# CLIAI/speaker-diarization-toolkit

Hardware: AMD Instinct MI355X
Metric: segment-embeddings/sec (higher is better)
Workload: dtype bf16; 1 GPU; config #2: 1k synthetic 2-s segments/GPU -> fbank -> ECAPA-TDNN C=1024 -> L2 -> cosine argmax vs 100 profiles; segments_per_gpu=1000, embed_dim=192, weights=random-init seed 0 (20.77 M params), parallelism=segments sharded x1, profiles replicated

## Files before the change

speaker-diarization-toolkit_amd/csrc/common.hpp:

```cpp
#pragma once
#include <hip/hip_runtime.h>
#include <stdint.h>
#include <stdio.h>
#include <vector>

#include "../../include/sdk_hip.h"

typedef __bf16 bf16_t;
typedef __bf16 bf16x8 __attribute__((ext_vector_type(8)));
typedef __bf16 bf16x4 __attribute__((ext_vector_type(4)));
typedef __bf16 bf16x2 __attribute__((ext_vector_type(2)));
typedef float f32x4 __attribute__((ext_vector_type(4)));
typedef float f32x16 __attribute__((ext_vector_type(16)));
typedef uint32_t u32x4 __attribute__((ext_vector_type(4)));
typedef uint32_t u32x2 __attribute__((ext_vector_type(2)));

struct sdk_prof_rec {
  int family;
  hipEvent_t a, b;
  double flops, bytes;
};
struct sdk_ctx {
  int device;
  int num_cu;
  hipDeviceProp_t prop;
  bool prof_on = false;
  bool no_chain_fusion = false;
  bool no_chain_two_per_cu = false;
  bool no_chain_packed = false;
  bool no_asp_packed = false;
  bool no_asp_seg = false;
  bool no_h_kblocked = false;
  int precision = 0;
  int aff_fast = 1;
  void* dbg_ptr = nullptr;
  void* gemm_clk_ptr = nullptr;
  void* gemm_stamps_ptr = nullptr;
  int hp_gemm_variant = 0;
  int matvec_variant = 0;
  int aff_boundary_pen = 0;
  int chol_pivot_rtol_ppb = 1000;
  int chol_shift_ppb = 0;
  bool ahc_distances_only = false;
  bool snorm_scores_only = false;
  int aff_variant = 0;
  std::vector<const void*> lds_optin;
  std::vector<sdk_prof_rec> prof;
};

int sdk_lds_optin(sdk_ctx* ctx, const void* func, int bytes);

int asp_fused_launch(sdk_ctx* ctx, const uint16_t* ah, int64_t ldah, const uint16_t* w2, const uint16_t* w2p, const float* b2,
                     const uint16_t* h, int64_t ldh, int B, int T, int C, int A, float* pooled, void* stream, bool kblocked = false, bool f16 = false);

int se_gate_residual_impl(sdk_ctx* ctx, const uint16_t* z, int64_t ldz, const uint16_t* x, int64_t ldx, const float* w1t, const float* b1, const float* w2t,
                          const float* b2, uint16_t* out, int64_t ldo, int B, int T, int C, int Cse, const float* mean_in, void* ws, size_t ws_bytes,
                          void* stream, bool f16);
int asp_stats_impl(sdk_ctx* ctx, const uint16_t* h, int64_t ldh, int B, int T, int C, float* out_ctx, void* stream, bool f16);
int asp_pool_impl(sdk_ctx* ctx, const float* logits, int64_t ldl, const uint16_t* h, int64_t ldh, int B, int T, int C, float* pooled, void* stream, bool f16);

int res2net_chain_launch(sdk_ctx* ctx, const uint16_t* U, int64_t ldu, uint16_t* R, int64_t ldr, const uint16_t* const* W,
                         const uint16_t* const* Wpk, const float* const* bias, const float* const* scale, const float* const* shift,
                         int nconv, int B, int T, int dil, void* stream, bool f16 = false);

int resnet_tstp_impl(sdk_ctx* ctx, const uint16_t* x, int B, int F, int T, int C, float* out, void* stream, bool f16);
int resnet_masked_tstp_impl(sdk_ctx* ctx, const uint16_t* x, int B, int F, int T, int C, int S, const float* w, const int32_t* valid, float* out,
                            void* stream, bool f16);
int resnet_zero_invalid_impl(sdk_ctx* ctx, float* emb, int n, int dim, const int32_t* valid, void* stream);

size_t ahc_workspace_bytes(const int32_t* offsets, int G);
int ahc_launch(sdk_ctx* ctx, const float* E, int ldE, int dim, const int32_t* offsets, int G, double* Z, int32_t* status, void* ws, void* stream);

struct ProfScope {
  sdk_ctx* c; hipStream_t s; size_t slot; bool on;
  ProfScope(sdk_ctx* ctx, void* stream, int family, double flops, double bytes) : c(ctx), s((hipStream_t)stream), slot(0), on(ctx && ctx->prof_on) {
    if (!on) return;
    sdk_prof_rec r{family, nullptr, nullptr, flops, bytes};
    (void)hipEventCreate(&r.a); (void)hipEventCreate(&r.b);
    (void)hipEventRecord(r.a, s);
    slot = c->prof.size();
    c->prof.push_back(r);
  }
  ~ProfScope() { if (on) (void)hipEventRecord(c->prof[slot].b, s); }
};

void sdk_set_error(const char* fmt, ...) __attribute__((format(printf, 1, 2)));

#define SDK_HIP_OK(expr)                                                              \
  do {                                                                                \
    hipError_t _e = (expr);                                                           \
    if (_e != hipSuccess) {                                                           \
      sdk_set_error("%s failed: %s (%s:%d)", #expr, hipGetErrorString(_e), __FILE__, __LINE__); \
      return 1;                                                                       \
    }                                                                                 \
  } while (0)

#define SDK_REQUIRE(cond, ...)            \
  do {                                    \
    if (!(cond)) {                        \
      sdk_set_error(__VA_ARGS__);         \
      return 2;                           \
    }                                     \
  } while (0)

#define SDK_LAUNCH_CHECK()                                                         \
  do {                                                                             \
    hipError_t _e = hipGetLastError();                                             \
    if (_e != hipSuccess) {                                                        \
      sdk_set_error("kernel launch failed: %s (%s:%d)", hipGetErrorString(_e), __FILE__, __LINE__); \
      return 1;                                                                    \
    }                                                                              \
  } while (0)

static inline int ceil_div(int a, int b) { return (a + b - 1) / b; }

__device__ __forceinline__ float bf16_to_f32(bf16_t v) { return (float)v; }
__device__ __forceinline__ bf16_t f32_to_bf16(float v) { return (bf16_t)v; }

__device__ __forceinline__ float bf16_bits_to_f32(uint32_t lo16) { return __uint_as_float(lo16 << 16); }

__device__ __forceinline__ void unpack8(const u32x4& v, float* f) {
#pragma unroll
  for (int i = 0; i < 4; ++i) {
    f[2 * i] = __uint_as_float(v[i] << 16);
    f[2 * i + 1] = __uint_as_float(v[i] & 0xffff0000u);
  }
}
__device__ __forceinline__ uint32_t pack2(float a, float b) {
  bf16x2 t;
  t[0] = (bf16_t)a;
  t[1] = (bf16_t)b;
  return __builtin_bit_cast(uint32_t, t);
}
typedef _Float16 f16x8_t __attribute__((ext_vector_type(8)));
typedef _Float16 f16x2_t __attribute__((ext_vector_type(2)));
__device__ __forceinline__ float sat_f16(float a) {
  const float c = fminf(fmaxf(a, -65504.f), 65504.f);
  return a != a ? a : c;
}
template <bool F16>
__device__ __forceinline__ uint32_t pack2t(float a, float b) {
  if constexpr (F16) {
    f16x2_t t;
    t[0] = (_Float16)sat_f16(a);
    t[1] = (_Float16)sat_f16(b);
    return __builtin_bit_cast(uint32_t, t);
  } else {
    return pack2(a, b);
  }
}
template <bool F16>
__device__ __forceinline__ void unpack8t(const u32x4& v, float* f) {
  if constexpr (F16) {
#pragma unroll
    for (int i = 0; i < 4; ++i) {
      const uint32_t w = v[i];
      const f16x2_t t = __builtin_bit_cast(f16x2_t, w);
      f[2 * i] = (float)t[0];
      f[2 * i + 1] = (float)t[1];
    }
  } else {
    unpack8(v, f);
  }
}

__device__ __forceinline__ u32x4 pack8(const float* f) {
  u32x4 v;
#pragma unroll
  for (int i = 0; i < 4; ++i) v[i] = pack2(f[2 * i], f[2 * i + 1]);
  return v;
}
template <bool F16>
__device__ __forceinline__ u32x4 pack8t(const float* f) {
  u32x4 v;
#pragma unroll
  for (int i = 0; i < 4; ++i) v[i] = pack2t<F16>(f[2 * i], f[2 * i + 1]);
  return v;
}
template <bool F16>
__device__ __forceinline__ float load1t(const bf16_t* q) {
  if constexpr (F16) return (float)*reinterpret_cast<const _Float16*>(q);
  else return bf16_to_f32(*q);
}
template <bool F16>
__device__ __forceinline__ f32x4 mfma_16x16x32(bf16x8 a, bf16x8 b, f32x4 c) {
  if constexpr (F16) return __builtin_amdgcn_mfma_f32_16x16x32_f16(__builtin_bit_cast(f16x8_t, a), __builtin_bit_cast(f16x8_t, b), c, 0, 0, 0);
  else return __builtin_amdgcn_mfma_f32_16x16x32_bf16(a, b, c, 0, 0, 0);
}
template <bool F16>
__device__ __forceinline__ f32x16 mfma_32x32x16(bf16x8 a, bf16x8 b, f32x16 c) {
  if constexpr (F16) return __builtin_amdgcn_mfma_f32_32x32x16_f16(__builtin_bit_cast(f16x8_t, a), __builtin_bit_cast(f16x8_t, b), c, 0, 0, 0);
  else return __builtin_amdgcn_mfma_f32_32x32x16_bf16(a, b, c, 0, 0, 0);
}

__device__ __forceinline__ float wave_sum(float v) {
#pragma unroll
  for (int o = 32; o > 0; o >>= 1) v += __shfl_xor(v, o, 64);
  return v;
}
__device__ __forceinline__ float wave_max(float v) {
#pragma unroll
  for (int o = 32; o > 0; o >>= 1) v = fmaxf(v, __shfl_xor(v, o, 64));
  return v;
}

__device__ __forceinline__ void lds_barrier() {
  asm volatile("s_waitcnt lgkmcnt(0)" ::: "memory");
  __builtin_amdgcn_s_barrier();
}

__device__ __forceinline__ float var_floor(float v) { return v < 1e-12f ? 1e-12f : v; }

__device__ __forceinline__ int reflect_idx(int t, int T) {
  t = t < 0 ? -t : t;
  return t >= T ? 2 * (T - 1) - t : t;
}

__device__ __forceinline__ int xcd_remap(int bid, int nwg) {
  const int q = nwg >> 3, r = nwg & 7, xcd = bid & 7, local = bid >> 3;
  const int base = xcd < r ? xcd * (q + 1) : r * (q + 1) + (xcd - r) * q;
  return base + local;
}
```

speaker-diarization-toolkit_amd/csrc/conv_gemm.hip:

```cpp
#include <stdlib.h>

#include <type_traits>

#include "common.hpp"
#ifndef SDK_GEMM_CHAIN2
#define SDK_GEMM_CHAIN2 2
#endif

namespace {

__device__ __forceinline__ float tanh_bf16(float x) { return 1.0f - __fdividef(2.0f, __expf(2.0f * x) + 1.0f); }

constexpr int BM = 128, BN = 128, BK = 64, NT = 256;
constexpr int LDS_AB = (BM + BN) * BK * 2;
constexpr int CT_STRIDE = (BN + 8) * 2;
constexpr int LDS_CT = BM * CT_STRIDE;
constexpr int LDS_BYTES = LDS_CT > LDS_AB ? LDS_CT : LDS_AB;

struct Params {
  const bf16_t* A; int64_t lda;
  const bf16_t* W;
  bf16_t* C; int64_t ldc;
  float* C32; int64_t ldc32;
  const float* bias; const float* scale; const float* shift;
  const float* ubias; int64_t ldub;
  const bf16_t* X2; int64_t ldx2;
  bf16_t* S; int64_t lds;
  int M, N, Cin, taps, dil, T;
  uint32_t flags;
  int tune;
  float* stats_part; int stats_mode;
  const bf16_t* A2; int64_t lda2;
  int64_t ablk, cblk;
  int tap_pack;
  unsigned long long* clk;
  unsigned long long* stamps;
};

template <bool F16>
__global__ __launch_bounds__(NT, 2) void conv_gemm_kernel(Params p) {
  extern __shared__ __attribute__((aligned(16))) char smem[];
  char* sA = smem;
  char* sB = smem + BM * BK * 2;

  const int tid = threadIdx.x;
  const int lane = tid & 63;
  const int wid = tid >> 6;
  const int wm = wid >> 1, wn = wid & 1;

  const int nbn = p.N / BN;
  const int nbm = (p.M + BM - 1) / BM;
  const int tile = xcd_remap(blockIdx.x, nbn * nbm);
  const int bn = tile % nbn, bm = tile / nbn;
  const int m0 = bm * BM, n0 = bn * BN;

  const int ch = tid & 7;
  const int r0 = tid >> 3;
  int segbase[4], tloc[4];
#pragma unroll
  for (int i = 0; i < 4; ++i) {
    int m = m0 + r0 + 32 * i;
    m = m < p.M ? m : p.M - 1;
    if (p.taps > 1) {
      const int b = m / p.T;
      segbase[i] = b * p.T;
      tloc[i] = m - b * p.T;
    } else {
      segbase[i] = m;
      tloc[i] = 0;
    }
  }
  const int cpt = p.tap_pack >> 3;
  const int cin_w = p.tap_pack ? BK : p.Cin;
  const int Ktot = p.tap_pack ? ((p.taps * p.tap_pack + BK - 1) / BK) * BK : p.taps * p.Cin;
  const bf16_t* wrow[4];
#pragma unroll
  for (int i = 0; i < 4; ++i) wrow[i] = p.W + (int64_t)(n0 + r0 + 32 * i) * Ktot + ch * 8;

  uint32_t lds_w[4];
#pragma unroll
  for (int i = 0; i < 4; ++i) {
    const int row = r0 + 32 * i;
    lds_w[i] = row * 128 + ((ch ^ (row & 7)) << 4);
  }

  const int ksteps_per_tap = cin_w / BK;
  const int nk = p.tap_pack ? Ktot / BK : p.taps * ksteps_per_tap;
  const int half = p.taps >> 1;

  u32x4 ra[4], rb[4], ra2[4];
  auto gload = [&](int s) {
    const int j = s / ksteps_per_tap;
    const int kc = (s - j * ksteps_per_tap) * BK;
    int off = (j - half) * p.dil, acol = kc + ch * 8;
    if (p.tap_pack) {
      const int g = s * 8 + ch;
      int tap = g / cpt;
      acol = (g - tap * cpt) * 8;
      if (tap >= p.taps) { tap = half; acol = 0; }
      off = (tap - half) * p.dil;
    }
#pragma unroll
    for (int i = 0; i < 4; ++i) {
      const int src = p.taps > 1 ? segbase[i] + reflect_idx(tloc[i] + off, p.T) : segbase[i];
      ra[i] = *reinterpret_cast<const u32x4*>(p.ablk ? p.A + (int64_t)(acol >> 6) * p.ablk + (int64_t)src * 64 + (acol & 63) : p.A + (int64_t)src * p.lda + acol);
      rb[i] = *reinterpret_cast<const u32x4*>(wrow[i] + j * cin_w + kc);
      if (p.A2) ra2[i] = *reinterpret_cast<const u32x4*>(p.A2 + (int64_t)src * p.lda2 + acol);
    }
  };

  f32x4 acc[4][4];
#pragma unroll
  for (int mi = 0; mi < 4; ++mi)
#pragma unroll
    for (int ni = 0; ni < 4; ++ni) acc[mi][ni] = f32x4{0.f, 0.f, 0.f, 0.f};

  const int fr = lane & 15, fq = lane >> 4;
  uint32_t a_off[4], b_off[4];
#pragma unroll
  for (int i = 0; i < 4; ++i) {
    a_off[i] = (wm * 64 + i * 16 + fr) * 128;
    b_off[i] = (wn * 64 + i * 16 + fr) * 128;
  }
  const int sw = lane & 7;

  gload(0);
  for (int s = 0; s < nk; ++s) {
#pragma unroll
    for (int i = 0; i < 4; ++i) {
      if (p.A2) {
        float fa[8], fb[8];
        unpack8t<F16>(ra[i], fa);
        unpack8t<F16>(ra2[i], fb);
#pragma unroll
        for (int e = 0; e < 8; ++e) fa[e] += fb[e];
        ra[i] = pack8t<F16>(fa);
      }
      *reinterpret_cast<u32x4*>(sA + lds_w[i]) = ra[i];
      *reinterpret_cast<u32x4*>(sB + lds_w[i]) = rb[i];
    }
    __syncthreads();
    if (s + 1 < nk) gload(s + 1);
#pragma unroll
    for (int ks = 0; ks < 2; ++ks) {
      const uint32_t coff = ((ks * 4 + fq) ^ sw) << 4;
      bf16x8 af[4], bfr[4];
#pragma unroll
      for (int i = 0; i < 4; ++i) {
        af[i] = *reinterpret_cast<const bf16x8*>(sA + a_off[i] + coff);
        bfr[i] = *reinterpret_cast<const bf16x8*>(sB + b_off[i] + coff);
      }
#pragma unroll
      for (int mi = 0; mi < 4; ++mi)
#pragma unroll
        for (int ni = 0; ni < 4; ++ni)
          acc[mi][ni] = mfma_16x16x32<F16>(af[mi], bfr[ni], acc[mi][ni]);
    }
    __syncthreads();
  }

  float cb[4], cs[4], ct[4];
#pragma unroll
  for (int ni = 0; ni < 4; ++ni) {
    const int col = n0 + wn * 64 + ni * 16 + fr;
    cb[ni] = p.bias ? p.bias[col] : 0.f;
    cs[ni] = p.scale ? p.scale[col] : 1.f;
    ct[ni] = p.shift ? p.shift[col] : 0.f;
  }
  const bool relu = p.flags & SDK_GEMM_RELU, tnh = p.flags & SDK_GEMM_TANH;
#pragma unroll
  for (int mi = 0; mi < 4; ++mi) {
#pragma unroll
    for (int r = 0; r < 4; ++r) {
      const int row = wm * 64 + mi * 16 + fq * 4 + r;
      const int m = m0 + row;
      const float* ub = nullptr;
      if (p.ubias) {
        const int mm = m < p.M ? m : p.M - 1;
        ub = p.ubias + (int64_t)(mm / p.T) * p.ldub;
      }
#pragma unroll
      for (int ni = 0; ni < 4; ++ni) {
        const int lc = wn * 64 + ni * 16 + fr;
        float v = acc[mi][ni][r] + cb[ni];
        if (ub) v += ub[n0 + lc];
        if (relu) v = fmaxf(v, 0.f);
        v = v * cs[ni] + ct[ni];
        if (tnh) v = tanh_bf16(v);
        if (p.C32 && m < p.M) p.C32[(int64_t)m * p.ldc32 + n0 + lc] = v;
        *reinterpret_cast<uint16_t*>(smem + row * CT_STRIDE + lc * 2) = (uint16_t)pack2t<F16>(v, 0.f);
      }
    }
  }
  __syncthreads();
  if (p.C || p.S) {
#pragma unroll
    for (int i = 0; i < 8; ++i) {
      const int id = tid + NT * i;
      const int row = id >> 4, cc = id & 15;
      const int m = m0 + row;
      if (m < p.M) {
        const u32x4 v = *reinterpret_cast<const u32x4*>(smem + row * CT_STRIDE + cc * 16);
        if (p.C) *reinterpret_cast<u32x4*>(p.C + (int64_t)m * p.ldc + n0 + cc * 8) = v;
        if (p.S) {
          const u32x4 x = *reinterpret_cast<const u32x4*>(p.X2 + (int64_t)m * p.ldx2 + n0 + cc * 8);
          float fv[8], fx[8];
          unpack8t<F16>(v, fv);
          unpack8t<F16>(x, fx);
#pragma unroll
          for (int e = 0; e < 8; ++e) fv[e] += fx[e];
          *reinterpret_cast<u32x4*>(p.S + (int64_t)m * p.lds + n0 + cc * 8) = pack8t<F16>(fv);
        }
      }
    }
  }
}

}

namespace {

constexpr int BM2 = 256, BN2 = 256, NT2 = 512;
constexpr int STAGE2 = (BM2 + BN2) * BK * 2;
constexpr int LDS2 = 2 * STAGE2;
constexpr int LDS2_PAR = LDS2 + 3 * BN2 * 4;
constexpr int LDS2_TOTAL = LDS2_PAR + 8 * 2 * BN2 * 4;
static_assert(BM2 * BN2 * 2 <= LDS2, "the bf16 image of a finished tile must fit in the two pipeline stages");

typedef const void __attribute__((address_space(1)))* gptr_t;
typedef void __attribute__((address_space(3)))* lptr_t;

template <bool TAPS, bool CKB = false, bool F16 = false>
__global__ __launch_bounds__(NT2, 2) void conv_gemm256_kernel(Params p) {
  extern __shared__ __attribute__((aligned(16))) char smem[];
  const int tid = threadIdx.x, lane = tid & 63, wid = tid >> 6;
  const unsigned long long clk_c0 = p.clk ? __builtin_amdgcn_s_memtime() : 0, clk_r0 = p.clk ? __builtin_amdgcn_s_memrealtime() : 0;
  const int wm = wid >> 2, wn = wid & 3;

  const int nbn = p.N / BN2;
  const int nbm = (p.M + BM2 - 1) / BM2;
  const int ntiles = nbn * nbm;
  const int cpt = p.tap_pack >> 3;
  const int cin_w = p.tap_pack ? BK : p.Cin;
  const int Ktot = p.tap_pack ? ((p.taps * p.tap_pack + BK - 1) / BK) * BK : p.taps * p.Cin;
  const int ksteps_per_tap = cin_w / BK;
  const int nk = p.tap_pack ? Ktot / BK : p.taps * ksteps_per_tap;
  const int half = p.taps >> 1;

  const int G = gridDim.x;
  const bool unit_order = !(p.tune & 64) && G == 256 && (nbn & 3) == 0 && nbm >= 64;
  const int xcd = blockIdx.x & 7, slot = blockIdx.x >> 3;
  const int nch = nbn >> 2, mg_full = nbm >> 3;
  const int full_units = mg_full * nch, R = full_units >> 3, rem_units = full_units - 8 * R;
  const int gm_tail = nbm & 7, tail_tiles = gm_tail * nbn;
  const int mt0 = unit_order && (8 * R) % nch == 0 ? ((8 * R) / nch) * 8 : 0;
  const int n_half_m = 2 * (nbm - mt0);
  const int half_cap = 32 / nbn;
  const bool half_tail = unit_order && !(p.tune & 512) && (8 * R) % nch == 0 && R > 0 && mt0 < nbm && n_half_m <= 8 * half_cap;
  const int nrounds = unit_order ? (half_tail ? R : R + (rem_units + (tail_tiles + 31) / 32 + 7) / 8) : (ntiles + G - 1) / G;
  auto tile_coords = [&](int i, int& tm0, int& tn0) -> bool {
    if (unit_order) {
      int u;
      if (i < R) {
        u = xcd * R + i;
      } else {
        const int q = (i - R) * 8 + xcd;
        if (q >= rem_units) {
          const int pj = (q - rem_units) * 32 + slot;
          if (pj >= tail_tiles) return false;
          tm0 = (mg_full * 8 + pj % gm_tail) * BM2;
          tn0 = (pj / gm_tail) * BN2;
          return true;
        }
        u = 8 * R + q;
      }
      const int mg = u / nch, ch = u - mg * nch;
      tm0 = (mg * 8 + (slot & 7)) * BM2;
      tn0 = (ch * 4 + (slot >> 3)) * BN2;
      return true;
    }
    const int vt = blockIdx.x + G * i;
    if (vt >= ntiles) return false;
    const int tile = xcd_remap(vt, ntiles);
    constexpr int GM = 8;
    const int per_group = GM * nbn;
    const int grp = tile / per_group, in_grp = tile - grp * per_group;
    const int gm = min(nbm - grp * GM, GM);
    tm0 = (grp * GM + in_grp % gm) * BM2;
    tn0 = (in_grp / gm) * BN2;
    return true;
  };

  const int rin = lane >> 3, pos = lane & 7;
  const int gch = (pos ^ rin) * 8;
  const int wu = __builtin_amdgcn_readfirstlane(wid);
  const bool a_nt = !TAPS && nbn <= 4;
  uint32_t aoff[4];
  int aseg0 = 0, atl0 = 0;
  uint32_t woff;
  auto setup_dma = [&](int tm0, int tn0, auto ap_c) {
    constexpr int AP = decltype(ap_c)::value;
    const int row = 8 * AP * wu + rin;
    if constexpr (TAPS) {
      const int mm = min(tm0 + row, p.M - 1);
      aseg0 = (mm / p.T) * p.T;
      atl0 = mm - aseg0;
    } else {
#pragma unroll
      for (int i = 0; i < AP; ++i) aoff[i] = ((uint32_t)min(tm0 + row + 8 * i, p.M - 1) * (uint32_t)p.lda + (uint32_t)gch) * 2u;
    }
    woff = ((uint32_t)(tn0 + 32 * wu + rin) * (uint32_t)Ktot + (uint32_t)gch) * 2u;
  };
  auto issue = [&](int t, int stage, auto ap_c) {
    constexpr int AP = decltype(ap_c)::value;
    const int j = t / ksteps_per_tap;
    const int kc = (t - j * ksteps_per_tap) * BK;
    char* sA = smem + stage * STAGE2 + (8 * AP * wu) * 128;
    char* sB = smem + stage * STAGE2 + BM2 * BK * 2 + (32 * wu) * 128;
    const char* abase = reinterpret_cast<const char*>(p.A + kc);
    if constexpr (TAPS) {
      int off = (j - half) * p.dil;
      uint32_t acol = (uint32_t)gch;
      if (p.tap_pack) {
        const int g = t * 8 + (gch >> 3);
        int tap = g / cpt;
        acol = (uint32_t)(g - tap * cpt) * 8u;
        if (tap >= p.taps) { tap = half; acol = 0; }
        off = (tap - half) * p.dil;
      }
#pragma unroll
      for (int i = 0; i < AP; ++i) {
        int tl = atl0 + 8 * i, sb = aseg0;
        if (tl >= p.T) { tl -= p.T; sb += p.T; }
        const uint32_t src = (uint32_t)min(sb + reflect_idx(tl + off, p.T), p.M - 1);
        __builtin_amdgcn_global_load_lds((gptr_t)(abase + (size_t)((src * (uint32_t)p.lda + acol) * 2u)), (lptr_t)(sA + i * 1024), 16, 0, 0);
      }
    } else if (a_nt) {
#pragma unroll
      for (int i = 0; i < AP; ++i)
        __builtin_amdgcn_global_load_lds((gptr_t)(abase + (size_t)aoff[i]), (lptr_t)(sA + i * 1024), 16, 0, 2);
    } else {
#pragma unroll
      for (int i = 0; i < AP; ++i)
// ... 429 lines not shown
        }
        v = v * qs[ni] + qt[ni];
        uint2 pk;
        pk.x = pack2t<F16>(v[0], v[1]);
        pk.y = pack2t<F16>(v[2], v[3]);
        const int u8 = (wn * 16 + ni * 4 + fq) ^ (fr << 1);
        *reinterpret_cast<uint2*>(rowp + u8 * 8) = pk;
      }
    }
    lds_barrier();
    {
      const int r0 = tid >> 5, cc = tid & 31;
      const char* src = smem + r0 * (BN2 * 2) + ((cc ^ (r0 & 15)) << 4);
      bf16_t* dst = CKB ? p.C + (int64_t)((n0 >> 6) + (cc >> 3)) * p.cblk + (int64_t)(m0 + r0) * 64 + (cc & 7) * 8
                        : p.C + (int64_t)(m0 + r0) * p.ldc + n0 + cc * 8;
      const int64_t ldc = CKB ? 64 : p.ldc;
      const int rows_left = p.M - m0 - r0;
#pragma unroll
      for (int i = 0; i < 8; ++i) {
        if (16 * i < rows_left) {
          const u32x4 v = *reinterpret_cast<const u32x4*>(src + i * 16 * (BN2 * 2));
          __builtin_nontemporal_store(v, reinterpret_cast<u32x4*>(dst + (int64_t)(16 * i) * ldc));
        }
      }
    }
    if (stats) tile_stats((m0 / BM2) * BM2, m0 & 128, 128, n0);
    stamp();
    }
  }
  if (p.clk && tid == 0 && blockIdx.x < 4096) {
    p.clk[blockIdx.x * 2] = __builtin_amdgcn_s_memtime() - clk_c0;
    p.clk[blockIdx.x * 2 + 1] = __builtin_amdgcn_s_memrealtime() - clk_r0;
  }
}

__global__ __launch_bounds__(256) void colstats_finish_kernel(const float* __restrict__ part, int M, int N, int T, int mode,
                                                             float* __restrict__ out) {
  const int b = blockIdx.x, n = blockIdx.y * 256 + threadIdx.x;
  if (n >= N) return;
  const int64_t nbm = (M + BM2 - 1) / BM2;
  const int r_lo = b * T, r_hi = (b + 1) * T - 1;
  float s = 0.f, q = 0.f;
  for (int t = r_lo / BM2; t <= r_hi / BM2; ++t) {
    const int slot = b - (t * BM2) / T;
    const float* ps = part + ((int64_t)(t * 2) * 3 + slot) * N + n;
    s += ps[0];
    s += ps[3 * (int64_t)N];
    if (mode == 2) {
      const float* pq = ps + nbm * 6 * N;
      q += pq[0];
      q += pq[3 * (int64_t)N];
    }
  }
  const float invT = 1.0f / (float)T;
  const float mean = s * invT;
  if (mode == 1) {
    out[(int64_t)b * N + n] = mean;
  } else {
    out[(int64_t)b * 2 * N + n] = mean;
    out[(int64_t)b * 2 * N + N + n] = sqrtf(var_floor(q * invT - mean * mean));
  }
}

int g_gemm_variant = -1;

}

extern "C" size_t sdk_conv_gemm_stats_bytes(int M, int N, int mode) {
  if (M <= 0 || N <= 0 || mode < 1 || mode > 2) return 0;
  return (size_t)((M + BM2 - 1) / BM2) * 6 * (size_t)N * sizeof(float) * (size_t)mode;
}

extern "C" int sdk_conv_gemm_stats_fusable(int M, int N, int T) {
  return ((g_gemm_variant < 0 ? 2 : g_gemm_variant) & 15) != 1 && N % BN2 == 0 && M >= BM2 && T >= 128;
}

extern "C" int sdk_colstats_finish(sdk_ctx* ctx, const float* stats_part, int M, int N, int T, int mode, float* out, void* stream) {
  SDK_REQUIRE(ctx && stats_part && out, "sdk_colstats_finish: null argument");
  SDK_REQUIRE(M > 0 && T > 0 && M % T == 0 && (mode == 1 || mode == 2), "sdk_colstats_finish: bad shape");
  hipLaunchKernelGGL(colstats_finish_kernel, dim3(M / T, ceil_div(N, 256)), dim3(256), 0, (hipStream_t)stream, stats_part, M, N, T, mode, out);
  SDK_LAUNCH_CHECK();
  return 0;
}

extern "C" int sdk_set_gemm_variant(int v) {
  g_gemm_variant = v;
  return 0;
}

extern "C" int sdk_conv_gemm(sdk_ctx* ctx, const sdk_conv_gemm_args* a, void* stream) {
  SDK_REQUIRE(ctx && a, "sdk_conv_gemm: null ctx/args");
  SDK_REQUIRE(a->A && a->W, "sdk_conv_gemm: A and W are required");
  SDK_REQUIRE(a->M > 0 && a->N > 0 && a->N % BN == 0, "sdk_conv_gemm: N=%d must be a positive multiple of %d", a->N, BN);
  const int pack = a->tap_pack;
  if (pack) {
    SDK_REQUIRE(pack > 0 && pack % 8 == 0 && a->taps > 1 && !a->A2 && a->Cin == pack, "sdk_conv_gemm: tap_pack=%d needs taps > 1, a multiple of 8 channels per tap, Cin == tap_pack and no A2", pack);
  } else
  SDK_REQUIRE(a->Cin > 0 && a->Cin % BK == 0, "sdk_conv_gemm: Cin=%d must be a multiple of %d", a->Cin, BK);
  SDK_REQUIRE(a->taps >= 1 && (a->taps & 1), "sdk_conv_gemm: taps=%d must be odd", a->taps);
  SDK_REQUIRE(a->T > 0 && a->M % a->T == 0, "sdk_conv_gemm: M=%d must be a multiple of T=%d", a->M, a->T);
  SDK_REQUIRE((int64_t)a->N * a->taps * a->Cin < (1ll << 31), "sdk_conv_gemm: weight matrix of %d x %d elements exceeds 2^31", a->N, a->taps * a->Cin);
  SDK_REQUIRE(a->taps == 1 || (a->taps / 2) * a->dil < a->T, "sdk_conv_gemm: segment of T=%d frames shorter than the conv halo %d", a->T, (a->taps / 2) * a->dil);
  const bool a_kb = (a->flags & SDK_GEMM_A_KBLOCKED) != 0, c_kb = (a->flags & SDK_GEMM_C_KBLOCKED) != 0, f16 = (a->flags & SDK_GEMM_F16) != 0;
  if (a_kb) SDK_REQUIRE(a->taps == 1 && !pack && !a->A2, "sdk_conv_gemm: a K-blocked A operand needs taps == 1, no tap packing and no A2");
  else
  SDK_REQUIRE(a->lda % 8 == 0 && a->lda >= a->Cin, "sdk_conv_gemm: lda=%lld must be >= Cin and a multiple of 8", (long long)a->lda);
  SDK_REQUIRE(((uintptr_t)a->A % 16) == 0 && ((uintptr_t)a->W % 16) == 0, "sdk_conv_gemm: A/W must be 16-byte aligned");
  SDK_REQUIRE(a->C || a->C32 || a->S, "sdk_conv_gemm: no output requested");
  if (a->C && !c_kb) SDK_REQUIRE(a->ldc % 8 == 0 && a->ldc >= a->N && ((uintptr_t)a->C % 16) == 0, "sdk_conv_gemm: bad C/ldc");
  if (c_kb) SDK_REQUIRE(a->C && ((uintptr_t)a->C % 16) == 0, "sdk_conv_gemm: a K-blocked output needs C (16-byte aligned)");
  if (a->S) SDK_REQUIRE(a->X2 && a->lds % 8 == 0 && a->ldx2 % 8 == 0 && ((uintptr_t)a->S % 16) == 0 && ((uintptr_t)a->X2 % 16) == 0, "sdk_conv_gemm: S needs X2 and 16-byte aligned rows");
  if (a->C32) SDK_REQUIRE(a->ldc32 >= a->N, "sdk_conv_gemm: bad ldc32");
  if (a->ubias) SDK_REQUIRE(a->ldub >= a->N, "sdk_conv_gemm: bad ldub");

  if (g_gemm_variant < 0) {
    const char* e = getenv("SDK_GEMM_VARIANT");
    g_gemm_variant = e ? atoi(e) : 2;
  }
  if (sdk_lds_optin(ctx, (const void*)conv_gemm256_kernel<false>, LDS2_TOTAL)) return 1;
  if (sdk_lds_optin(ctx, (const void*)conv_gemm256_kernel<true>, LDS2_TOTAL)) return 1;
  if (sdk_lds_optin(ctx, (const void*)conv_gemm256_kernel<false, true>, LDS2_TOTAL)) return 1;
  if (sdk_lds_optin(ctx, (const void*)conv_gemm256_kernel<false, false, true>, LDS2_TOTAL)) return 1;
  if (sdk_lds_optin(ctx, (const void*)conv_gemm256_kernel<true, false, true>, LDS2_TOTAL)) return 1;
  if (sdk_lds_optin(ctx, (const void*)conv_gemm256_kernel<false, true, true>, LDS2_TOTAL)) return 1;
  Params p;
  p.A = (const bf16_t*)a->A; p.lda = a->lda; p.W = (const bf16_t*)a->W;
  p.C = (bf16_t*)a->C; p.ldc = a->ldc; p.C32 = a->C32; p.ldc32 = a->ldc32;
  p.bias = a->bias; p.scale = a->scale; p.shift = a->shift; p.ubias = a->ubias; p.ldub = a->ldub;
  p.X2 = (const bf16_t*)a->X2; p.ldx2 = a->ldx2; p.S = (bf16_t*)a->S; p.lds = a->lds;
  p.M = a->M; p.N = a->N; p.Cin = a->Cin; p.taps = a->taps; p.dil = a->dil; p.T = a->T; p.flags = a->flags;
  p.tune = g_gemm_variant / 16;
  p.stats_part = nullptr; p.stats_mode = 0;
  p.A2 = (const bf16_t*)a->A2; p.lda2 = a->lda2;
  p.tap_pack = pack;
  p.ablk = a_kb ? (int64_t)a->M * 64 : 0;
  p.cblk = c_kb ? (int64_t)a->M * 64 : 0;
  p.clk = (unsigned long long*)ctx->gemm_clk_ptr;
  p.stamps = (unsigned long long*)ctx->gemm_stamps_ptr;
  if (a->A2) SDK_REQUIRE(a->lda2 % 8 == 0 && a->lda2 >= a->Cin && ((uintptr_t)a->A2 % 16) == 0, "sdk_conv_gemm: bad A2/lda2");

  const double kk = pack ? (double)(((a->taps * pack + BK - 1) / BK) * BK) : (double)a->taps * a->Cin;
  const bool use256 = !a_kb && ((g_gemm_variant & 15) != 1 || c_kb) && a->N % BN2 == 0 && a->M >= BM2 && !a->A2 && a->C && !a->C32 && !a->S &&
                      !a->ubias && !(a->flags & SDK_GEMM_TANH) && (a->taps == 1 || a->T >= 64) &&
                      (uint64_t)a->M * (uint64_t)a->lda * 2u < (1ull << 32);
  ProfScope ps(ctx, stream, use256 ? SDK_K_CONV_GEMM256 : SDK_K_CONV_GEMM, 2.0 * a->M * a->N * kk,
               2.0 * a->M * a->Cin + 2.0 * a->N * kk + (a->C ? 2.0 : 0.0) * a->M * a->N + (a->C32 ? 4.0 : 0.0) * a->M * a->N +
                   (a->S ? 4.0 : 0.0) * a->M * a->N);
  if (c_kb) SDK_REQUIRE(use256 && a->taps == 1, "sdk_conv_gemm: a K-blocked output needs the plain-layer shape of the 256^2 kernel (taps == 1, N %% 256 == 0, M >= 256, bf16 output only)");
  if (a->stats_mode) {
    SDK_REQUIRE(a->stats_mode == 1 || a->stats_mode == 2, "sdk_conv_gemm: stats_mode=%d", a->stats_mode);
    SDK_REQUIRE(use256 && a->T >= 128 && a->stats_part && a->C, "sdk_conv_gemm: fused column statistics need the 256^2 kernel (N %% 256 == 0, M >= 256), T >= 128 and a bf16 output");
    p.stats_part = a->stats_part; p.stats_mode = a->stats_mode;
  }
  if (use256) {
    const int ntiles = (a->N / BN2) * ceil_div(a->M, BM2);
    const int cus = ctx->num_cu > 0 ? (ctx->num_cu / 8) * 8 : 256;
    const int grid = (p.tune & 8) ? ntiles : (ntiles < cus ? ntiles : cus);
    if (f16) {
      void (*kern)(Params) = conv_gemm256_kernel<false, false, true>;
      if (c_kb) kern = conv_gemm256_kernel<false, true, true>;
      else if (p.taps > 1) kern = conv_gemm256_kernel<true, false, true>;
      hipLaunchKernelGGL(kern, dim3(grid), dim3(NT2), LDS2_TOTAL, (hipStream_t)stream, p);
    } else if (c_kb)
      hipLaunchKernelGGL((conv_gemm256_kernel<false, true>), dim3(grid), dim3(NT2), LDS2_TOTAL, (hipStream_t)stream, p);
    else
      hipLaunchKernelGGL(p.taps > 1 ? conv_gemm256_kernel<true> : conv_gemm256_kernel<false>, dim3(grid), dim3(NT2), LDS2_TOTAL, (hipStream_t)stream, p);
  } else {
    hipLaunchKernelGGL(f16 ? conv_gemm_kernel<true> : conv_gemm_kernel<false>, dim3((a->N / BN) * ceil_div(a->M, BM)), dim3(NT), LDS_BYTES, (hipStream_t)stream, p);
  }
  SDK_LAUNCH_CHECK();
  return 0;
}
```

speaker-diarization-toolkit_amd/csrc/sdk_api.hip:

```cpp
#include <stdarg.h>
#include <string.h>

#include "common.hpp"
#include "ecapa_layout.h"
#include "hp.hpp"

static thread_local char g_err[512] = "";

void sdk_set_error(const char* fmt, ...) {
  va_list ap;
  va_start(ap, fmt);
  vsnprintf(g_err, sizeof(g_err), fmt, ap);
  va_end(ap);
}

extern "C" const char* sdk_last_error(void) { return g_err; }
extern "C" int sdk_abi_version(void) { return SDK_ABI_VERSION; }

extern "C" int sdk_init(int device, sdk_ctx** out) {
  SDK_REQUIRE(out, "sdk_init: out is null");
  *out = nullptr;
  int n = 0;
  hipError_t e = hipGetDeviceCount(&n);
  if (e != hipSuccess || n <= 0) {
    sdk_set_error("sdk_init: no HIP device available (%s); this library has no CPU fallback",
                  e != hipSuccess ? hipGetErrorString(e) : "device count is 0");
    return 1;
  }
  SDK_REQUIRE(device >= 0 && device < n, "sdk_init: device %d out of range (0..%d)", device, n - 1);
  sdk_ctx* c = new sdk_ctx();
  c->device = device;
  if (hipGetDeviceProperties(&c->prop, device) != hipSuccess) {
    delete c;
    sdk_set_error("sdk_init: hipGetDeviceProperties failed");
    return 1;
  }
  if (strncmp(c->prop.gcnArchName, "gfx950", 6) != 0) {
    sdk_set_error("sdk_init: device %d is %s; libsdk_hip.so carries gfx950 (MI355X) code objects only", device,
                  c->prop.gcnArchName);
    delete c;
    return 1;
  }
  c->num_cu = c->prop.multiProcessorCount;
  SDK_HIP_OK(hipSetDevice(device));
  *out = c;
  return 0;
}

int sdk_lds_optin(sdk_ctx* ctx, const void* func, int bytes) {
  for (const void* f : ctx->lds_optin)
    if (f == func) return 0;
  SDK_HIP_OK(hipSetDevice(ctx->device));
  SDK_HIP_OK(hipFuncSetAttribute(func, hipFuncAttributeMaxDynamicSharedMemorySize, bytes));
  ctx->lds_optin.push_back(func);
  return 0;
}

extern "C" int sdk_device_malloc(sdk_ctx* ctx, size_t bytes, void** out) {
  SDK_REQUIRE(ctx && out, "sdk_device_malloc: null argument");
  *out = nullptr;
  SDK_HIP_OK(hipSetDevice(ctx->device));
  SDK_HIP_OK(hipMalloc(out, bytes ? bytes : 1));
  return 0;
}
extern "C" int sdk_device_free(sdk_ctx* ctx, void* p) {
  SDK_REQUIRE(ctx, "sdk_device_free: null context");
  if (p) SDK_HIP_OK(hipFree(p));
  return 0;
}
extern "C" int sdk_memcpy(sdk_ctx* ctx, void* dst, const void* src, size_t bytes, int kind, void* stream) {
  SDK_REQUIRE(ctx && (bytes == 0 || (dst && src)), "sdk_memcpy: null argument");
  SDK_REQUIRE(kind >= 1 && kind <= 3, "sdk_memcpy: kind=%d (1 = host to device, 2 = device to host, 3 = device to device)", kind);
  if (!bytes) return 0;
  const hipMemcpyKind k = kind == 1 ? hipMemcpyHostToDevice : kind == 2 ? hipMemcpyDeviceToHost : hipMemcpyDeviceToDevice;
  SDK_HIP_OK(hipMemcpyAsync(dst, src, bytes, k, (hipStream_t)stream));
  SDK_HIP_OK(hipStreamSynchronize((hipStream_t)stream));
  return 0;
}
extern "C" int sdk_stream_synchronize(sdk_ctx* ctx, void* stream) {
  SDK_REQUIRE(ctx, "sdk_stream_synchronize: null context");
  SDK_HIP_OK(hipStreamSynchronize((hipStream_t)stream));
  return 0;
}

extern "C" int sdk_shutdown(sdk_ctx* ctx) {
  delete ctx;
  return 0;
}

extern "C" int sdk_get_device_info(sdk_ctx* ctx, sdk_device_info* out) {
  SDK_REQUIRE(ctx && out, "sdk_get_device_info: null argument");
  memset(out, 0, sizeof(*out));
  out->device = ctx->device;
  out->compute_units = ctx->prop.multiProcessorCount;
  out->clock_khz = ctx->prop.clockRate;
  out->wavefront_size = ctx->prop.warpSize;
  out->hbm_bytes = ctx->prop.totalGlobalMem;
  strncpy(out->name, ctx->prop.name, sizeof(out->name) - 1);
  strncpy(out->arch, ctx->prop.gcnArchName, sizeof(out->arch) - 1);
  return 0;
}

extern "C" int sdk_set_option(sdk_ctx* ctx, const char* name, int value) {
  SDK_REQUIRE(ctx && name, "sdk_set_option: null argument");
  if (strcmp(name, "res2net_chain_fusion") == 0) { ctx->no_chain_fusion = value == 0; return 0; }
  if (strcmp(name, "res2net_packed_weights") == 0) { ctx->no_chain_packed = value == 0; return 0; }
  if (strcmp(name, "res2net_two_per_cu") == 0) { ctx->no_chain_two_per_cu = value == 0; return 0; }
  if (strcmp(name, "asp_packed_weights") == 0) { ctx->no_asp_packed = value == 0; return 0; }
  if (strcmp(name, "asp_per_segment") == 0) { ctx->no_asp_seg = value == 0; return 0; }
  if (strcmp(name, "h_kblocked") == 0) { ctx->no_h_kblocked = value == 0; return 0; }
  if (strcmp(name, "precision") == 0) {
    SDK_REQUIRE(value >= 0 && value <= 2, "sdk_set_option: precision must be 0 (bf16 operands), 1 (fp16 hi+lo planes) or 2 (one fp16 plane), got %d", value);
    ctx->precision = value;
    return 0;
  }
  if (strcmp(name, "gemm_variant") == 0) return sdk_set_gemm_variant(value);
  if (strcmp(name, "affinity_fast_path") == 0) { ctx->aff_fast = value; return 0; }
  if (strcmp(name, "affinity_variant") == 0) { ctx->aff_variant = value; return 0; }
  if (strcmp(name, "affinity_boundary_penalty") == 0) { ctx->aff_boundary_pen = value < 0 ? 0 : value; return 0; }
  if (strcmp(name, "matvec_variant") == 0) { ctx->matvec_variant = value; return 0; }
  if (strcmp(name, "hp_gemm_variant") == 0) { ctx->hp_gemm_variant = value; return 0; }
  if (strcmp(name, "affinity_whole_groups") == 0) return 0;
  if (strcmp(name, "chol_pivot_rtol_ppb") == 0) { ctx->chol_pivot_rtol_ppb = value < 0 ? 0 : value; return 0; }
  if (strcmp(name, "chol_shift_ppb") == 0) { ctx->chol_shift_ppb = value < 0 ? 0 : value; return 0; }
  if (strcmp(name, "ahc_distances_only") == 0) { ctx->ahc_distances_only = value != 0; return 0; }
  if (strcmp(name, "snorm_scores_only") == 0) { ctx->snorm_scores_only = value != 0; return 0; }
  sdk_set_error("sdk_set_option: unknown option '%s'", name);
  return 2;
}

extern "C" int sdk_debug_set_ptr(sdk_ctx* ctx, const char* name, void* p) {
  SDK_REQUIRE(ctx && name, "sdk_debug_set_ptr: null argument");
  if (strcmp(name, "stamps") == 0) { ctx->dbg_ptr = p; return 0; }
  if (strcmp(name, "gemm_clock") == 0) { ctx->gemm_clk_ptr = p; return 0; }
  if (strcmp(name, "gemm_stamps") == 0) { ctx->gemm_stamps_ptr = p; return 0; }
  sdk_set_error("sdk_debug_set_ptr: unknown name '%s'", name);
  return 2;
}

extern "C" int sdk_profile_begin(sdk_ctx* ctx) {
  SDK_REQUIRE(ctx, "sdk_profile_begin: null ctx");
  for (auto& r : ctx->prof) { (void)hipEventDestroy(r.a); (void)hipEventDestroy(r.b); }
  ctx->prof.clear();
  ctx->prof_on = true;
  return 0;
}

extern "C" int sdk_profile_end(sdk_ctx* ctx, sdk_profile_report* out) {
  SDK_REQUIRE(ctx && out, "sdk_profile_end: null argument");
  ctx->prof_on = false;
  memset(out, 0, sizeof(*out));
  SDK_HIP_OK(hipDeviceSynchronize());
  for (auto& r : ctx->prof) {
    float ms = 0.f;
    SDK_HIP_OK(hipEventElapsedTime(&ms, r.a, r.b));
    if (r.family >= 0 && r.family < SDK_K_COUNT) {
      out->launches[r.family] += 1;
      out->ms[r.family] += ms;
      out->flops[r.family] += r.flops;
      out->bytes[r.family] += r.bytes;
    }
    (void)hipEventDestroy(r.a);
    (void)hipEventDestroy(r.b);
  }
  ctx->prof.clear();
  return 0;
}

namespace {

inline size_t a256(size_t v) { return (v + 255) & ~(size_t)255; }

struct FwdWs {
  uint16_t *X0, *U, *R, *Z, *Sa, *Sb, *CAT, *H, *AH;
  float *ctx, *ubias, *logits, *pooled, *se, *stats, *mean;
};

size_t fwd_layout(const sdk_ecapa_desc* d, int B, int T, char* base, FwdWs* w) {
  const size_t M = (size_t)B * T, C = d->channels, Cm = d->mfa_channels, S = d->sub_channels, A = d->attn_channels;
  size_t off = 0;
  auto take = [&](size_t bytes) { char* p = base ? base + off : nullptr; off += a256(bytes); return p; };
  char* x0 = take(M * C * 2);
  char* u = take(M * C * 2);
  char* r = take(M * C * 2);
  char* z = take(M * C * 2);
  char* sa = take(M * S * 2);
  char* sb = take(M * S * 2);
  char* cat = take(M * Cm * 2);
  char* h = take(M * Cm * 2);
  char* ah = take(M * A * 2);
  char* cx = take((size_t)B * 2 * Cm * 4);
  char* ub = take((size_t)B * A * 4);
  const bool fused_asp = A == 128 && T <= sdk_asp_fused_max_frames();
  char* lg = take(fused_asp ? 256 : M * Cm * 4);
  char* po = take((size_t)B * 2 * Cm * 4);
  char* se = take(sdk_se_workspace_bytes(B, (int)C, d->se_channels));
  char* stp = take(sdk_conv_gemm_stats_bytes((int)M, (int)Cm, 2));
  char* mn = take((size_t)B * C * 4);
  if (w) { w->se = (float*)se; w->stats = (float*)stp; w->mean = (float*)mn; }
  if (w) {
    w->X0 = (uint16_t*)x0; w->U = (uint16_t*)u; w->R = (uint16_t*)r; w->Z = (uint16_t*)z;
    w->Sa = (uint16_t*)sa; w->Sb = (uint16_t*)sb; w->CAT = (uint16_t*)cat; w->H = (uint16_t*)h; w->AH = (uint16_t*)ah;
    w->ctx = (float*)cx; w->ubias = (float*)ub; w->logits = (float*)lg; w->pooled = (float*)po;
  }
  return off;
}

struct FwdWsHp {
  uint16_t *X0, *U, *R, *Z, *Sa, *Sb, *CAT, *H, *AH;
  float *ctx, *ubias, *logits, *pooled, *mean, *hid, *gate;
};

size_t fwd_layout_hp(const sdk_ecapa_desc* d, int B, int T, char* base, FwdWsHp* w) {
  const size_t M = (size_t)B * T, C = d->channels, Cm = d->mfa_channels, S = d->sub_channels, A = d->attn_channels;
  size_t off = 0;
  auto take = [&](size_t bytes) { char* p = base ? base + off : nullptr; off += a256(bytes); return p; };
  char* x0 = take(M * C * 4);
  char* u = take(M * C * 4);
  char* r = take(M * C * 4);
  char* z = take(M * C * 4);
  char* sa = take(M * S * 4);
  char* sb = take(M * S * 4);
  char* cat = take(M * Cm * 4);
  char* h = take(M * Cm * 4);
  char* ah = take(M * A * 4);
  char* cx = take((size_t)B * 2 * Cm * 4);
  char* ub = take((size_t)B * A * 4);
  char* lg = take(M * Cm * 4);
  char* po = take((size_t)B * 2 * Cm * 4);
  char* mn = take((size_t)B * C * 4);
  char* hd = take((size_t)B * d->se_channels * 4);
  char* gt = take((size_t)B * C * 4);
  if (w) {
    w->X0 = (uint16_t*)x0; w->U = (uint16_t*)u; w->R = (uint16_t*)r; w->Z = (uint16_t*)z; w->Sa = (uint16_t*)sa; w->Sb = (uint16_t*)sb;
    w->CAT = (uint16_t*)cat; w->H = (uint16_t*)h; w->AH = (uint16_t*)ah; w->ctx = (float*)cx; w->ubias = (float*)ub; w->logits = (float*)lg;
    w->pooled = (float*)po; w->mean = (float*)mn; w->hid = (float*)hd; w->gate = (float*)gt;
  }
  return off;
}

int check_desc(const sdk_ecapa_desc* d) {
  SDK_REQUIRE(d, "ecapa desc is null");
  SDK_REQUIRE(d->n_blocks >= 1 && d->n_blocks <= 4, "ecapa desc: n_blocks=%d", d->n_blocks);
  SDK_REQUIRE(d->channels % 128 == 0 && d->mfa_channels == d->n_blocks * d->channels, "ecapa desc: channels=%d mfa=%d", d->channels, d->mfa_channels);
  SDK_REQUIRE(d->scale >= 2 && d->sub_channels * d->scale == d->channels && d->sub_channels % 128 == 0, "ecapa desc: res2net scale=%d sub=%d", d->scale, d->sub_channels);
  SDK_REQUIRE(d->attn_channels % 128 == 0 && d->n_mels_padded % (d->precision == 1 ? 32 : 64) == 0, "ecapa desc: attn=%d mels=%d", d->attn_channels, d->n_mels_padded);
  SDK_REQUIRE((d->kernel0 & 1) == 1, "ecapa desc: kernel0=%d must be odd", d->kernel0);
  SDK_REQUIRE(d->precision >= 0 && d->precision <= 2, "ecapa desc: precision=%d", d->precision);
  return 0;
}

int ecapa_forward_hp(sdk_ctx* ctx, const void* wblob, const sdk_ecapa_desc* d, const uint16_t* feats, int ldf, int B, int T, void* ws,
                     float* emb, void* stream) {
  FwdWsHp w;
  fwd_layout_hp(d, B, T, (char*)ws, &w);
  const char* wb = (const char*)wblob;
  auto P16 = [&](int slot) -> const uint16_t* { return d->off[slot] < 0 ? nullptr : (const uint16_t*)(wb + d->off[slot]); };
  auto P32 = [&](int slot) -> const float* { return d->off[slot] < 0 ? nullptr : (const float*)(wb + d->off[slot]); };
  const int M = B * T, C = d->channels, Cm = d->mfa_channels, S = d->sub_channels, A = d->attn_channels;
  const int flo = ldf >> 1;
  SDK_REQUIRE(ldf % 16 == 0 && flo >= d->n_mels_padded, "sdk_ecapa_forward: precise mode takes feature planes, ldf=%d must be >= 2 x %d", ldf, d->n_mels_padded);

  auto tdnn = [&](const uint16_t* Ain, int64_t lda, int64_t a_lo, int Cin, int taps, int dil, int slot, int N, uint16_t* Cout, int64_t ldc, int64_t c_lo,
// ... 505 lines not shown
```

Baseline: 119,400 segment-embeddings/sec.

## Add persistent streaming GEMM kernel for ASP attention-hidden layer

Adds a dedicated persistent kernel for the attention-hidden GEMM (N=128, K-blocked A). Each block owns a contiguous range of rows and walks 256-row tiles through a three-stage global_load_lds ring, with the per-segment bias staged in LDS. The goal is to replace the generic 128x128 conv GEMM for this skinny-N shape, cutting launch-tail waste and improving load/compute overlap. The epilogue is factored into a shared helper. It adds code complexity and a new path that depends on the K-blocked layout and on M*128 fitting in 32 bits.

```diff
diff --git a/speaker-diarization-toolkit_amd/csrc/asp_hidden.hip b/speaker-diarization-toolkit_amd/csrc/asp_hidden.hip
--- /dev/null
+++ b/speaker-diarization-toolkit_amd/csrc/asp_hidden.hip
@@ -0,0 +1,186 @@
+#include "common.hpp"
+
+namespace {
+
+constexpr int HM = 256, HN = 128, HK = 64, HNT = 512;
+constexpr int H_STAGE_A = HM * HK * 2;
+constexpr int H_STAGE = H_STAGE_A + HN * HK * 2;
+constexpr int H_RING = 3 * H_STAGE;
+constexpr int H_UB_SEGS = 8;
+constexpr int H_LDS = H_RING + H_UB_SEGS * HN * 4;
+constexpr int H_CT = (HN + 8) * 2;
+static_assert(HM * H_CT <= H_RING, "the 2-byte image of a finished tile must fit in the ring");
+
+struct HParams {
+  const bf16_t* A; const bf16_t* W;
+  bf16_t* C; int64_t ldc;
+  const float* bias; const float* scale; const float* shift;
+  const float* ubias; int64_t ldub;
+  int M, K, T;
+  uint32_t flags;
+};
+
+typedef const void __attribute__((address_space(1)))* gptr_t;
+typedef void __attribute__((address_space(3)))* lptr_t;
+
+template <bool F16>
+__global__ __launch_bounds__(HNT, 2) void asp_hidden_kernel(HParams p) {
+  extern __shared__ __attribute__((aligned(16))) char smem[];
+  const int tid = threadIdx.x, lane = tid & 63;
+  const int wu = __builtin_amdgcn_readfirstlane(tid >> 6);
+  const int wm = wu >> 1, wn = wu & 1;
+  const int nk = p.K / HK;
+
+  const int units = (p.M + 127) >> 7, G = gridDim.x, b = blockIdx.x;
+  const int uq = units / G, ur = units - uq * G;
+  const int u0 = b * uq + min(b, ur), nu = uq + (b < ur ? 1 : 0);
+  const int mbeg = u0 * 128, mend = min((u0 + nu) * 128, p.M);
+
+  const int rin = lane >> 3, pos = lane & 7;
+  const uint32_t gch = (uint32_t)((pos ^ rin) << 4);
+  const int64_t ablk = (int64_t)p.M * 128;
+  uint32_t aoff[4], woff[2];
+#pragma unroll
+  for (int j = 0; j < 2; ++j) woff[j] = (uint32_t)(16 * wu + 8 * j + rin) * (uint32_t)p.K * 2u + gch;
+  auto issue = [&](int t, int stage) {
+    char* sA = smem + stage * H_STAGE + (32 * wu) * 128;
+    char* sB = smem + stage * H_STAGE + H_STAGE_A + (16 * wu) * 128;
+    const char* abase = reinterpret_cast<const char*>(p.A) + (int64_t)t * ablk;
+    const char* wbase = reinterpret_cast<const char*>(p.W) + (size_t)t * 128;
+#pragma unroll
+    for (int i = 0; i < 4; ++i) __builtin_amdgcn_global_load_lds((gptr_t)(abase + (size_t)aoff[i]), (lptr_t)(sA + i * 1024), 16, 0, 2);
+#pragma unroll
+    for (int j = 0; j < 2; ++j) __builtin_amdgcn_global_load_lds((gptr_t)(wbase + (size_t)woff[j]), (lptr_t)(sB + j * 1024), 16, 0, 0);
+  };
+
+  const int fr = lane & 15, fq = lane >> 4, sw = lane & 7;
+  uint32_t a_off[4], b_off[4];
+#pragma unroll
+  for (int i = 0; i < 4; ++i) {
+    a_off[i] = (wm * 64 + i * 16 + fr) * 128;
+    b_off[i] = H_STAGE_A + (wn * 64 + i * 16 + fr) * 128;
+  }
+
+  float cb[4], cs[4], ct[4];
+#pragma unroll
+  for (int ni = 0; ni < 4; ++ni) {
+    const int col = wn * 64 + ni * 16 + fr;
+    cb[ni] = p.bias ? p.bias[col] : 0.f;
+    cs[ni] = p.scale ? p.scale[col] : 1.f;
+    ct[ni] = p.shift ? p.shift[col] : 0.f;
+  }
+  const bool relu = p.flags & SDK_GEMM_RELU, tnh = p.flags & SDK_GEMM_TANH;
+
+  for (int m0 = mbeg; m0 < mend; m0 += HM) {
+    const bool active = wm < 2 || m0 + 128 < mend;
+#pragma unroll
+    for (int i = 0; i < 4; ++i) aoff[i] = (uint32_t)min(m0 + 32 * wu + 8 * i + rin, mend - 1) * 128u + gch;
+
+    f32x4 acc[4][4];
+#pragma unroll
+    for (int mi = 0; mi < 4; ++mi)
+#pragma unroll
+      for (int ni = 0; ni < 4; ++ni) acc[mi][ni] = f32x4{0.f, 0.f, 0.f, 0.f};
+
+    const int s0 = m0 / p.T;
+    if (p.ubias) {
+      const float* src = p.ubias + (int64_t)min(s0 + wu, p.M / p.T - 1) * p.ldub + lane;
+#pragma unroll
+      for (int j = 0; j < 2; ++j) __builtin_amdgcn_global_load_lds((gptr_t)(src + 64 * j), (lptr_t)(smem + H_RING + wu * (HN * 4) + j * 256), 4, 0, 0);
+    }
+    issue(0, 0);
+    if (nk > 1) issue(1, 1);
+    int st = 0, st2 = 2;
+    for (int t = 0; t < nk; ++t) {
+      if (t == 0 || t + 1 >= nk) asm volatile("s_waitcnt vmcnt(0) lgkmcnt(0)" ::: "memory");
+      else asm volatile("s_waitcnt vmcnt(6) lgkmcnt(0)" ::: "memory");
+      __builtin_amdgcn_s_barrier();
+      if (t + 2 < nk) issue(t + 2, st2);
+      if (active) {
+        const char* sp = smem + st * H_STAGE;
+#pragma unroll
+        for (int ks = 0; ks < 2; ++ks) {
+          const uint32_t coff = ((ks * 4 + fq) ^ sw) << 4;
+          bf16x8 af[4], bfr[4];
+#pragma unroll
+          for (int i = 0; i < 4; ++i) {
+            af[i] = *reinterpret_cast<const bf16x8*>(sp + a_off[i] + coff);
+            bfr[i] = *reinterpret_cast<const bf16x8*>(sp + b_off[i] + coff);
+          }
+#pragma unroll
+          for (int mi = 0; mi < 4; ++mi)
+#pragma unroll
+            for (int ni = 0; ni < 4; ++ni) acc[mi][ni] = mfma_16x16x32<F16>(af[mi], bfr[ni], acc[mi][ni]);
+        }
+      }
+      st = st == 2 ? 0 : st + 1;
+      st2 = st2 == 2 ? 0 : st2 + 1;
+    }
+
+    lds_barrier();
+    if (active) {
+      const bool has_ub = p.ubias != nullptr;
+      const float* ubt = reinterpret_cast<const float*>(smem + H_RING);
+#pragma unroll
+      for (int mi = 0; mi < 4; ++mi) {
+        float ubv[4][4];
+#pragma unroll
+        for (int r = 0; r < 4; ++r) {
+          const int m = min(m0 + wm * 64 + mi * 16 + fq * 4 + r, p.M - 1);
+          const int sl = has_ub ? min(m / p.T - s0, H_UB_SEGS - 1) : 0;
+#pragma unroll
+          for (int ni = 0; ni < 4; ++ni) ubv[r][ni] = has_ub ? ubt[sl * HN + wn * 64 + ni * 16 + fr] : 0.f;
+        }
+#pragma unroll
+        for (int r = 0; r < 4; ++r) {
+          const int row = wm * 64 + mi * 16 + fq * 4 + r;
+#pragma unroll
+          for (int ni = 0; ni < 4; ++ni) {
+            const int lc = wn * 64 + ni * 16 + fr;
+            float v;
+            const uint16_t h = gemm_epilogue_elem<F16>(acc[mi][ni][r], cb[ni], has_ub, ubv[r][ni], relu, cs[ni], ct[ni], tnh, v);
+            *reinterpret_cast<uint16_t*>(smem + row * H_CT + lc * 2) = h;
+          }
+        }
+      }
+    }
+    lds_barrier();
+#pragma unroll
+    for (int i = 0; i < 8; ++i) {
+      const int id = tid + HNT * i;
+      const int row = id >> 4, cc = id & 15;
+      const int m = m0 + row;
+      if (m < mend) {
+        const u32x4 v = *reinterpret_cast<const u32x4*>(smem + row * H_CT + cc * 16);
+        *reinterpret_cast<u32x4*>(p.C + (int64_t)m * p.ldc + cc * 8) = v;
+      }
+    }
+    lds_barrier();
+  }
+}
+
+}
+
+bool asp_hidden_ok(const sdk_ctx* ctx, const sdk_conv_gemm_args* a) {
+  const uint32_t known = SDK_GEMM_RELU | SDK_GEMM_TANH | SDK_GEMM_A_KBLOCKED | SDK_GEMM_F16;
+  return !ctx->no_asp_hidden_stream && (a->flags & SDK_GEMM_A_KBLOCKED) && !(a->flags & ~known) && a->taps == 1 && a->N == HN && a->Cin >= HK &&
+         a->Cin % HK == 0 && a->M >= HM && a->C && !a->C32 && !a->S && !a->A2 && !a->tap_pack && !a->stats_mode &&
+         (uint64_t)a->M * 128u < (1ull << 32) &&
+         (!a->ubias || a->T >= 64);
+}
+
+int asp_hidden_launch(sdk_ctx* ctx, const sdk_conv_gemm_args* a, void* stream) {
+  SDK_REQUIRE(asp_hidden_ok(ctx, a), "asp_hidden_launch: not the attention-hidden shape");
+  const bool f16 = (a->flags & SDK_GEMM_F16) != 0;
+  void (*kern)(HParams) = f16 ? asp_hidden_kernel<true> : asp_hidden_kernel<false>;
+  if (sdk_lds_optin(ctx, (const void*)kern, H_LDS)) return 1;
+  HParams p;
+  p.A = (const bf16_t*)a->A; p.W = (const bf16_t*)a->W; p.C = (bf16_t*)a->C; p.ldc = a->ldc;
+  p.bias = a->bias; p.scale = a->scale; p.shift = a->shift; p.ubias = a->ubias; p.ldub = a->ldub;
+  p.M = a->M; p.K = a->Cin; p.T = a->T; p.flags = a->flags;
+  const int units = ceil_div(a->M, 128);
+  const int cus = ctx->num_cu > 0 ? (ctx->num_cu / 8) * 8 : 256;
+  hipLaunchKernelGGL(kern, dim3(units < cus ? units : cus), dim3(HNT), H_LDS, (hipStream_t)stream, p);
+  SDK_LAUNCH_CHECK();
+  return 0;
+}
diff --git a/speaker-diarization-toolkit_amd/csrc/common.hpp b/speaker-diarization-toolkit_amd/csrc/common.hpp
--- a/speaker-diarization-toolkit_amd/csrc/common.hpp
+++ b/speaker-diarization-toolkit_amd/csrc/common.hpp
@@ -31,6 +31,7 @@
   bool no_asp_packed = false;
   bool no_asp_seg = false;
   bool no_h_kblocked = false;
+  bool no_asp_hidden_stream = false;
   int precision = 0;
   int aff_fast = 1;
   void* dbg_ptr = nullptr;
@@ -59,6 +60,9 @@
 int asp_stats_impl(sdk_ctx* ctx, const uint16_t* h, int64_t ldh, int B, int T, int C, float* out_ctx, void* stream, bool f16);
 int asp_pool_impl(sdk_ctx* ctx, const float* logits, int64_t ldl, const uint16_t* h, int64_t ldh, int B, int T, int C, float* pooled, void* stream, bool f16);
 
+bool asp_hidden_ok(const sdk_ctx* ctx, const sdk_conv_gemm_args* a);
+int asp_hidden_launch(sdk_ctx* ctx, const sdk_conv_gemm_args* a, void* stream);
+
 int res2net_chain_launch(sdk_ctx* ctx, const uint16_t* U, int64_t ldu, uint16_t* R, int64_t ldr, const uint16_t* const* W,
                          const uint16_t* const* Wpk, const float* const* bias, const float* const* scale, const float* const* shift,
                          int nconv, int B, int T, int dil, void* stream, bool f16 = false);
@@ -193,6 +197,18 @@
   else return __builtin_amdgcn_mfma_f32_32x32x16_bf16(a, b, c, 0, 0, 0);
 }
 
+__device__ __forceinline__ float tanh_bf16(float x) { return 1.0f - __fdividef(2.0f, __expf(2.0f * x) + 1.0f); }
+
+template <bool F16>
+__device__ __forceinline__ uint16_t gemm_epilogue_elem(float acc, float cb, bool has_ub, float ubv, bool relu, float cs, float ct, bool tnh, float& v) {
+  v = acc + cb;
+  if (has_ub) v += ubv;
+  if (relu) v = fmaxf(v, 0.f);
+  v = v * cs + ct;
+  if (tnh) v = tanh_bf16(v);
+  return (uint16_t)pack2t<F16>(v, 0.f);
+}
+
 __device__ __forceinline__ float wave_sum(float v) {
 #pragma unroll
   for (int o = 32; o > 0; o >>= 1) v += __shfl_xor(v, o, 64);
diff --git a/speaker-diarization-toolkit_amd/csrc/conv_gemm.hip b/speaker-diarization-toolkit_amd/csrc/conv_gemm.hip
--- a/speaker-diarization-toolkit_amd/csrc/conv_gemm.hip
+++ b/speaker-diarization-toolkit_amd/csrc/conv_gemm.hip
@@ -8,8 +8,6 @@
 #endif
 
 namespace {
-
-__device__ __forceinline__ float tanh_bf16(float x) { return 1.0f - __fdividef(2.0f, __expf(2.0f * x) + 1.0f); }
 
 constexpr int BM = 128, BN = 128, BK = 64, NT = 256;
 constexpr int LDS_AB = (BM + BN) * BK * 2;
@@ -182,13 +180,10 @@
 #pragma unroll
       for (int ni = 0; ni < 4; ++ni) {
         const int lc = wn * 64 + ni * 16 + fr;
-        float v = acc[mi][ni][r] + cb[ni];
-        if (ub) v += ub[n0 + lc];
-        if (relu) v = fmaxf(v, 0.f);
-        v = v * cs[ni] + ct[ni];
-        if (tnh) v = tanh_bf16(v);
+        float v;
+        const uint16_t h = gemm_epilogue_elem<F16>(acc[mi][ni][r], cb[ni], ub != nullptr, ub ? ub[n0 + lc] : 0.f, relu, cs[ni], ct[ni], tnh, v);
         if (p.C32 && m < p.M) p.C32[(int64_t)m * p.ldc32 + n0 + lc] = v;
-        *reinterpret_cast<uint16_t*>(smem + row * CT_STRIDE + lc * 2) = (uint16_t)pack2t<F16>(v, 0.f);
+        *reinterpret_cast<uint16_t*>(smem + row * CT_STRIDE + lc * 2) = h;
       }
     }
   }
@@ -924,6 +919,9 @@
     SDK_REQUIRE(use256 && a->T >= 128 && a->stats_part && a->C, "sdk_conv_gemm: fused column statistics need the 256^2 kernel (N %% 256 == 0, M >= 256), T >= 128 and a bf16 output");
     p.stats_part = a->stats_part; p.stats_mode = a->stats_mode;
   }
+  if (!use256 && (g_gemm_variant & 15) != 1 && asp_hidden_ok(ctx, a)) {
+    return asp_hidden_launch(ctx, a, stream);
+  }
   if (use256) {
     const int ntiles = (a->N / BN2) * ceil_div(a->M, BM2);
     const int cus = ctx->num_cu > 0 ? (ctx->num_cu / 8) * 8 : 256;
diff --git a/speaker-diarization-toolkit_amd/csrc/sdk_api.hip b/speaker-diarization-toolkit_amd/csrc/sdk_api.hip
--- a/speaker-diarization-toolkit_amd/csrc/sdk_api.hip
+++ b/speaker-diarization-toolkit_amd/csrc/sdk_api.hip
@@ -109,6 +109,7 @@
   if (strcmp(name, "asp_packed_weights") == 0) { ctx->no_asp_packed = value == 0; return 0; }
   if (strcmp(name, "asp_per_segment") == 0) { ctx->no_asp_seg = value == 0; return 0; }
   if (strcmp(name, "h_kblocked") == 0) { ctx->no_h_kblocked = value == 0; return 0; }
+  if (strcmp(name, "asp_hidden_stream") == 0) { ctx->no_asp_hidden_stream = value == 0; return 0; }
   if (strcmp(name, "precision") == 0) {
     SDK_REQUIRE(value >= 0 && value <= 2, "sdk_set_option: precision must be 0 (bf16 operands), 1 (fp16 hi+lo planes) or 2 (one fp16 plane), got %d", value);
     ctx->precision = value;
```

New measurement: 121,200 segment-embeddings/sec (median of 5 runs). +1.5%, better.
